# gvtulder/elasticdeform

Hardware: AMD Instinct MI355X
Metric: Mvoxels/s fwd+grad, 256^3 fp32 order=3 (higher is better)
Workload: dtype f32; 1 GPU; cfg2: 3D 256x256x256 float32, 5x5x5 grid sigma 5, order 3, mode mirror, prefilter on, deform_grid + deform_grid_gradient per step, one volume per GPU; parallelism=1 volume per GPU, no collective

## Files before the change

### elasticdeform_amd/csrc/deform_k1z.hip

```cpp
#include <hip/hip_runtime.h>

#include <cstring>
#include <type_traits>

#include "ed_device.h"
#include "ed_gridfilter.h"
#include "ed_params.h"
#include "ed_tile.h"
#include "ed_workspace.h"
#include "ed_zwalk.h"

namespace ed {
namespace tile {

#ifdef EDHIP_K1_STATS
__device__ unsigned long long g_k1z_stats[8];
#define ZSTAT(K, N) atomicAdd(&g_k1z_stats[K], (unsigned long long)(N))
#else
#define ZSTAT(K, N) do { } while (0)
#endif

namespace {


// ... 13 lines not shown
typedef int zv8i __attribute__((ext_vector_type(8)));
typedef const __attribute__((address_space(4))) zv8i* crec_p;
__device__ __forceinline__ ZRecU zrec_unpack(const zv8i& v)
{
    ZRecU r;
    r.b0z = v[0];
    r.b0y = v[1];
    r.b0x = v[2];
    r.flags = v[3];
    r.pitch = (v[3] >> 8) & 255;
    r.ez = v[4] & 1023;
    r.ey = (v[4] >> 10) & 1023;
    r.ex = (int)((unsigned)v[4] >> 20);
    r.goff = v[5];
    r.plane = r.ey * r.pitch;
    return r;
}
__device__ __forceinline__ ZRecU zrec_load(crec_p p)
{
    const zv8i v = *p;
    return zrec_unpack(v);
}

__host__ __device__ __forceinline__ int zctl(int parity, int list, int xcd) { return (parity * 2 + list) * 8 + xcd; }

#define ED_RED6(CTRL)                                      \
    "v_min_i32_dpp %0, %0, %0 " CTRL "\n\t"                \
    "v_min_i32_dpp %1, %1, %1 " CTRL "\n\t"                \
    "v_min_i32_dpp %2, %2, %2 " CTRL "\n\t"                \
    "v_max_i32_dpp %3, %3, %3 " CTRL "\n\t"                \
    "v_max_i32_dpp %4, %4, %4 " CTRL "\n\t"                \
    "v_max_i32_dpp %5, %5, %5 " CTRL "\n\t"
__device__ __forceinline__ void zrow_box(int (&lo)[3], int (&hi)[3])
{
    asm volatile("s_nop 1\n\t"
                 ED_RED6("quad_perm:[1,0,3,2] row_mask:0xf bank_mask:0xf")
                 ED_RED6("quad_perm:[2,3,0,1] row_mask:0xf bank_mask:0xf")
                 ED_RED6("row_half_mirror row_mask:0xf bank_mask:0xf")
                 ED_RED6("row_mirror row_mask:0xf bank_mask:0xf")
                 : "+v"(lo[0]), "+v"(lo[1]), "+v"(lo[2]), "+v"(hi[0]), "+v"(hi[1]), "+v"(hi[2]));
}
#undef ED_RED6
__device__ __forceinline__ int zuni(int v) { return __builtin_amdgcn_readfirstlane(v); }
__device__ __forceinline__ void zlds_barrier() { asm volatile("s_waitcnt lgkmcnt(0)\n\ts_barrier" ::: "memory"); }
__device__ __forceinline__ void zdma_barrier() { asm volatile("s_waitcnt vmcnt(0) lgkmcnt(0)\n\ts_barrier" ::: "memory"); }
__device__ __forceinline__ void zglds16(const float* g, float* lds)
{
    __builtin_amdgcn_global_load_lds((const __attribute__((address_space(1))) void*)g,
                                     (__attribute__((address_space(3))) void*)lds, 16, 0, 0);
}
template <bool OUT16>
__device__ __forceinline__ void zstore_out(float* img, long long off, float val, int io16)
{
    if constexpr (OUT16)
        reinterpret_cast<unsigned short*>(img)[off] = (unsigned short)narrow16(val, io16);
    else
        __builtin_nontemporal_store(val, img + off);
}

__device__ __forceinline__ void zaxis_entry(const GridGeom& g, int a, int oi, double* w, int* idx)
{
    const double cp = control_coordinate(g.ncp[a], (int64_t)oi + g.off[a], g.in_len[a]);
    const int64_t start = window_start(cp, 3);
    const bool edge = start < 0 || start + 3 >= g.ncp[a];
    spline_weights(cp, 3, w);
// ... 3 lines not shown
}

constexpr int kGeoBlock = 256;
constexpr int kGeoWaves = kGeoBlock / 64;
__global__ __launch_bounds__(kGeoBlock) void k1z_geo_kernel(const GridGeom g, const HotGeom hg, const ZGeom zg,
                                                          const GridPrefilter gp)
{
    extern __shared__ __attribute__((aligned(16))) char smem[];
    const int tid = threadIdx.x;
    const int lane = tid & 63;
    const int wave = zuni(tid >> 6);
    const int sample = blockIdx.y;
    const int ncpz = (int)g.ncp[0], ncpy = (int)g.ncp[1], ncpx = (int)g.ncp[2];
    const int nyx = ncpy * ncpx;
    const int ngrid = 3 * ncpz * nyx;
    double* sG = reinterpret_cast<double*>(smem);
    double* sR = sG + ngrid;
    AxTab* sAx = reinterpret_cast<AxTab*>(sR + 64 * ncpz * 3);
    double* sMax = reinterpret_cast<double*>(sAx + 16);
    AxTab* sZ = reinterpret_cast<AxTab*>(sMax + 3 * kGeoWaves);
    int* sCls = reinterpret_cast<int*>(sZ + 4 * hg.tiles[0]);
    int* sBox = sCls + hg.tiles[0];
    int* sCnt = sBox + 64 * hg.tiles[0];
    if ((int)blockIdx.x >= hg.tiles[1] * hg.tiles[2]) {
        const long long nfill = (long long)(gridDim.x - hg.tiles[1] * hg.tiles[2]) * kGeoBlock;
        const long long me = (long long)(blockIdx.x - hg.tiles[1] * hg.tiles[2]) * kGeoBlock + tid;
        const long long n16 = zg.zero_bytes >> 4;
        int4* p16 = reinterpret_cast<int4*>(zg.zero_ptr);
        for (long long i = me; i < n16; i += nfill)
            p16[i] = make_int4(0, 0, 0, 0);
        if (me < (zg.zero_bytes & 15))
            zg.zero_ptr[(n16 << 4) + me] = 0;
        return;
    }
    const int ty = blockIdx.x / hg.tiles[2], tx = blockIdx.x - ty * hg.tiles[2];
    if (ED_DBG(hg.dbg, 1 << 23))
        return;
#ifdef EDHIP_EXPERIMENTS
#define ZTICK(K) do { if (hg.dbgbuf && tid == 0) hg.dbgbuf[(size_t)(blockIdx.x + blockIdx.y * gridDim.x) * 16 + (K)] = __builtin_readcyclecounter(); } while (0)
#else
#define ZTICK(K) do { } while (0)
#endif
    ZTICK(0);

    if (gp.total > 0 && !ED_DBG(hg.dbg, 1 << 28)) {
        grid_prefilter_in_lds<kGeoBlock>(gp, sG, tid);
        if (blockIdx.x == 0 && sample == 0)
            for (int e = tid; e < gp.total; e += kGeoBlock)
                store_cast(gp.out + (int64_t)e * gp.elem_size, gp.dtype, sG[e]);
    } else {
        const char* disp = g.disp + (int64_t)sample * zg.disp_bstride;
        for (int e = tid; e < ngrid; e += kGeoBlock) {
            const int h = e / (ncpz * nyx), r = e - h * (ncpz * nyx);
            const int j0 = r / nyx, j = r - j0 * nyx;
            const int j1 = j / ncpx, j2 = j - j1 * ncpx;
            sG[e] = load_as_double(disp + g.disp_stride[0] * h + g.disp_stride[1] * j0 + g.disp_stride[2] * j1 +
                                       g.disp_stride[3] * j2, g.disp_dtype);
        }
        __syncthreads();
    }
    ZTICK(1);
    if (blockIdx.x == 0 && sample == 0 && tid == 0 && zg.hint) {
        if (zg.hint_host)
            __hip_atomic_store(zg.hint_host, ((unsigned long long)(unsigned)zg.hint[1] << 32) | (unsigned)zg.hint[0],
                               __ATOMIC_RELAXED, __HIP_MEMORY_SCOPE_SYSTEM);
        zg.hint[0] = 0;
        zg.hint[1] = (int)zg.hint_seq;
    }
    for (int h = 0; h < 3 && !ED_DBG(hg.dbg, 1 << 29); ++h) {
        double m = 0.0;
        for (int e = tid; e < ncpz * nyx; e += kGeoBlock)
            m = fmax(m, fabs(sG[h * ncpz * nyx + e]));
        for (int sh = 32; sh >= 1; sh >>= 1)
            m = fmax(m, __shfl_xor(m, sh));
        if (lane == 0)
            sMax[h * kGeoWaves + wave] = m;
    }
    ZTICK(2);
    if (tid < 16 && !ED_DBG(hg.dbg, 1 << 30)) {
        const int a = tid < 8 ? 1 : 2;
        const int oi = min((tid < 8 ? ty : tx) * kT + (tid & 7), hg.out_len[a] - 1);
        AxTab t;
        zaxis_entry(g, a, oi, t.w, t.idx);
        sAx[tid] = t;
    }
    for (int e = tid; e < 4 * hg.tiles[0] && !zg.tables_only && !ED_DBG(hg.dbg, 1 << 26); e += kGeoBlock) {
        const int tz = e >> 2, nz = min(kT, hg.out_len[0] - tz * kT);
        AxTab t;
        zaxis_entry(g, 0, tz * kT + ((e & 3) * (nz - 1)) / 3, t.w, t.idx);
        sZ[e] = t;
    }
    if (blockIdx.x == 0 && sample == 0 && hg.nstep) {
        for (long long ss = tid; ss < hg.nsteps; ss += kGeoBlock) {
            long long vol_off = 0, img_off = 0, r = ss;
            for (int l = 0; l < hg.nstep; ++l) {
                const long long q = r / hg.step_len[l];
                const long long c = r - q * hg.step_len[l];
                vol_off += hg.vol_step[l] * c;
                img_off += hg.img_step[l] * c;
                r = q;
            }
            zg.steps[2 * ss] = vol_off;
            zg.steps[2 * ss + 1] = img_off;
        }
    }
    if (blockIdx.x == 0 && sample == 0 && tid == 0) {
        ZGen* zn = reinterpret_cast<ZGen*>(zg.zgen);
        for (int h = 0; h < 3; ++h) {
            zn->in_len[h] = hg.in_len[h];
            zn->out_len[h] = hg.out_len[h];
            zn->off[h] = hg.off[h];
            zn->period[h] = hg.period[h];
            zn->inv_period[h] = hg.inv_period[h];
            zn->offd[h] = (double)hg.off[h];
        }
        for (int k = 0; k < 12; ++k)
            zn->aff[k] = hg.affine[k];
        zn->mode = hg.mode;
        zn->cval = hg.cval;
        zn->hint = hg.hint;
    }
    if (blockIdx.x == 0 && sample == 0) {
        AxTab* zt = const_cast<AxTab*>(zg.zt);
        for (int oz = tid; oz < hg.out_len[0]; oz += kGeoBlock) {
            AxTab t;
            zaxis_entry(g, 0, oz, t.w, t.idx);
#pragma unroll
            for (int l = 0; l < 4; ++l)
                t.idx[l] *= 32;
            zt[oz] = t;
        }
    }
    __syncthreads();
    ZTICK(3);
    double slack[3];
#pragma unroll
    for (int h = 0; h < 3; ++h) {
        double m = 0.0;
        for (int w = 0; w < kGeoWaves; ++w)
            m = fmax(m, sMax[h * kGeoWaves + w]);
        const double sl = zg.slack_scale * m;
        slack[h] = sl >= 0.02 ? (sl <= 0.75 ? sl : 0.75) : 0.02;
    }
    ZTICK(4);
    if (!ED_DBG(hg.dbg, 1 << 25)) {
        const int col = tid & 63;
        const AxTab ay = sAx[col >> 3];
        const AxTab ax = sAx[8 + (col & 7)];
        int rowoff[4];
#pragma unroll
        for (int ly = 0; ly < 4; ++ly)
            rowoff[ly] = ay.idx[ly] * ncpx;
        for (int r = tid >> 6; r < ncpz * 3; r += kGeoWaves) {
            const int kz = r / 3, h = r - kz * 3;
            const double* gp0 = sG + (h * ncpz + kz) * nyx;
            double acc = 0.0;
#pragma unroll
            for (int ly = 0; ly < 4; ++ly) {
                const double* row = gp0 + rowoff[ly];
                double t = ax.w[0] * row[ax.idx[0]];
#pragma unroll
                for (int lx = 1; lx < 4; ++lx)
                    t = fma(ax.w[lx], row[ax.idx[lx]], t);
                acc = fma(ay.w[ly], t, acc);
            }
            sR[col * (ncpz * 3) + r] = acc;
        }
        __syncthreads();
        double* rg = const_cast<double*>(zg.r) + (int64_t)sample * zg.r_bstride;
        const int rowlen = 8 * 4 * ncpz;
        for (int e = tid; e < 8 * rowlen; e += kGeoBlock) {
            const int py = e / rowlen, j = e - py * rowlen;
            const int px = j / (4 * ncpz), jj = j - px * (4 * ncpz);
            const int kz = jj >> 2, h = jj & 3;
            const int oy = ty * kT + py, ox = tx * kT + px;
            if (oy < hg.out_len[1] && ox < hg.out_len[2])
                rg[((int64_t)oy * hg.out_len[2] + ox) * (4 * ncpz) + jj] = h < 3 ? sR[(py * 8 + px) * (ncpz * 3) + kz * 3 + h] : 0.0;
        }
    }
    if (zg.tables_only)
        return;
    __syncthreads();
    ZTICK(5);
    const int order = zg.order;
    const int H = order / 2, NT = order + 1, kPadX = NT & 1;
    const int ny = min(kT, hg.out_len[1] - ty * kT), nx = min(kT, hg.out_len[2] - tx * kT);
    const int py = (((lane >> 2) & 3) * (ny - 1)) / 3, px = ((lane & 3) * (nx - 1)) / 3;
    const double* rc = sR + (py * 8 + px) * (ncpz * 3);
    for (int tz = wave; tz < hg.tiles[0] && !ED_DBG(hg.dbg, 1 << 24); tz += kGeoWaves) {
        const int nz = min(kT, hg.out_len[0] - tz * kT);
        const int pz = ((lane >> 4) * (nz - 1)) / 3;
        const int o[3] = {tz * kT + pz, ty * kT + py, tx * kT + px};
        const AxTab& ze = sZ[tz * 4 + (lane >> 4)];
        double d[3];
#pragma unroll
        for (int h = 0; h < 3; ++h) {
            d[h] = ze.w[0] * rc[ze.idx[0] * 3 + h];
#pragma unroll
            for (int l = 1; l < 4; ++l)
                d[h] = fma(ze.w[l], rc[ze.idx[l] * 3 + h], d[h]);
        }
        double c[3];
        int lo[3], hi[3];
#pragma unroll
        for (int h = 0; h < 3; ++h) {
// ... 32 lines not shown
                    m = map_coordinate_fast(m, hg.in_len[h], hg.mode, hg.period[h], hg.inv_period[h]);
                cst = cst || !(m > -1.0);
                const double mr = (order & 1) ? m : m + 0.5;
                lo[h] = (int)floor(mr - slack[h]);
                hi[h] = (int)floor(mr + slack[h]);
            }
            if (cst) {
#pragma unroll
                for (int h = 0; h < 3; ++h) {
                    lo[h] = 0x7fffffff;
                    hi[h] = (int)0x80000000;
                }
            }
            zrow_box(lo, hi);
            if ((lane & 15) == 0) {
#pragma unroll
                for (int h = 0; h < 3; ++h) {
                    dst[32 + h] = lo[h];
                    dst[36 + h] = hi[h];
                }
            }
        }
    }
    __syncthreads();
    ZTICK(6);
    for (int tz = tid; tz < hg.tiles[0] && !ED_DBG(hg.dbg, 1 << 27); tz += kGeoBlock) {
        const int tile_id = sample * hg.ntiles + (tz * hg.tiles[1] + ty) * hg.tiles[2] + tx;
        int cls = 0;
        bool hint0 = false, half_fit[2] = {false, false};
#pragma unroll 1
        for (int part = 0; part < 3; ++part) {
            const int* sb = sBox + tz * 64;
            const bool fast = sb[3] != 0;
            const int r0 = part == 2 ? 2 : 0, r1 = part == 1 ? 2 : 3;
            int blo[3], bhi[3];
            bool any = true;
#pragma unroll
            for (int h = 0; h < 3; ++h) {
                int rlo = 0x7fffffff, rhi = (int)0x80000000, lo = 0x7fffffff, hi = (int)0x80000000;
                for (int r = r0; r <= r1; ++r) {
                    rlo = min(rlo, sb[r * 8 + h]);
                    rhi = max(rhi, sb[r * 8 + 4 + h]);
                    lo = min(lo, sb[(fast ? 0 : 32) + r * 8 + h]);
                    hi = max(hi, sb[(fast ? 0 : 32) + r * 8 + 4 + h]);
                }
                if (!fast) {
                    any = any && hi >= lo;
// ... 36 lines not shown
                dst[0] = w0;
                dst[1] = w1;
                if (hg.boxes) {
                    int* bx = hg.boxes + (size_t)tile_id * 8;
#pragma unroll
                    for (int h = 0; h < 3; ++h) {
                        bx[h] = blo[h];
                        bx[3 + h] = bhi[h] - ((h == 2 && any) ? kPadX : 0);
                    }
                }
                if (cls != 3)
                    break;
            } else {
                half_fit[part - 1] = fits || !any;
                int4* dst = reinterpret_cast<int4*>(zg.recs_half + ((size_t)tile_id * 2 + (part - 1)) * 8);
                dst[0] = w0;
                dst[1] = w1;
            }
        }
        const bool split = cls == 3 && half_fit[0] && half_fit[1];
        ZSTAT(cls == 3 ? (split ? 6 : 5) : (cls == 1 ? 3 : 4), 1);
        sCls[tz] = cls | (split ? 4 : 0) | (hint0 ? 8 : 0);
    }
    __syncthreads();
    ZTICK(7);
    {
        const int zstrips = (hg.tiles[0] + zg.strip_tiles - 1) / zg.strip_tiles;
        if (tid < 4)
            sCnt[tid] = 0;
        __syncthreads();
        int slotG = -1, slotF = -1, sidv = 0;
        if (tid < zstrips) {
            int info = 0;
            bool g = false, f = false;
            for (int k = 0; k < zg.strip_tiles && tid * zg.strip_tiles + k < hg.tiles[0]; ++k) {
                const int c = sCls[tid * zg.strip_tiles + k];
                info |= c << (4 * k);
                g = g || (c & 3) == 2 || (c & 7) == 7;
                f = f || (c & 7) == 3;
            }
            const size_t sid = (size_t)sample * zg.nstrips + ((size_t)tid * hg.tiles[1] + ty) * hg.tiles[2] + tx;
            sidv = (int)sid;
            zg.sinfo[sid] = info;
            zg.missed[sid] = f ? 2 : 0;
            if (g)
                slotG = atomicAdd(&sCnt[0], 1);
            if (f)
                slotF = atomicAdd(&sCnt[1], 1);
        }
        __syncthreads();
        const int xcd = (tx + ty + sample) & 7;
        if (tid == 0) {
            sCnt[2] = sCnt[0] ? atomicAdd(&zg.ctl[zctl(zg.parity, 0, xcd)], sCnt[0]) : 0;
            sCnt[3] = sCnt[1] ? atomicAdd(&zg.ctl[zctl(zg.parity, 1, xcd)], sCnt[1]) : 0;
        }
        if (blockIdx.x == 0 && sample == 0 && tid < 16)
            zg.ctl[zctl(1 - zg.parity, tid >> 3, tid & 7)] = 0;
        __syncthreads();
        if (slotG >= 0)
            zg.list_g[(size_t)(sCnt[2] + slotG) * 8 + xcd] = sidv;
        if (slotF >= 0)
            zg.list_f[(size_t)(sCnt[3] + slotF) * 8 + xcd] = sidv;
    }
    ZTICK(8);
#undef ZTICK
}


struct ZVox {
    int addr[2];
    float frac[2][3];
    int flg;
};
struct ZStrip {
    int tz0, ty, tx, ntile, sample, id;
};
__device__ __forceinline__ bool k1z_strip(int total_strips, int nstrips, int tiles_z, int tiles_y, int tiles_x, int strip_tiles, int deal,
                                          ZStrip& sp, int b)
{
    const int x = b & 7, j = b >> 3;
    const int r = j / deal;
    int s = (r * 8 + ((x + r) & 7)) * deal + (j - r * deal);
    if (s >= total_strips)
        return false;
    sp.id = s;
    sp.sample = s / nstrips;
    s -= sp.sample * nstrips;
    sp.tx = s % tiles_x;
    s /= tiles_x;
    sp.ty = s % tiles_y;
    sp.tz0 = (s / tiles_y) * strip_tiles;
    sp.ntile = min(strip_tiles, tiles_z - sp.tz0);
    return true;
}
inline unsigned k1z_grid(int total_strips, int deal)
{
    const int chunks = (total_strips + deal - 1) / deal;
    return (unsigned)(((chunks + 7) / 8) * 8 * deal);
}

template <int ORDER, int PITCH>
__device__ __forceinline__ float k1z_gather(const float* bp, int plane, int pitch_rt, const float* w0, const float* w1, const float* w2)
{
    constexpr int NT = ORDER + 1;
    constexpr int NTX = NT + (NT & 1);
    float a0 = 0.f;
#pragma unroll
    for (int l0 = 0; l0 < NT; ++l0) {
        const float* pp = bp + l0 * plane;
        float a1 = 0.f;
#pragma unroll
        for (int l1 = 0; l1 < NT; ++l1) {
            const float* rp = pp + l1 * (PITCH ? PITCH : pitch_rt);
            float a2 = 0.f;
#pragma unroll
            for (int l2 = 0; l2 < NTX; l2 += 2) {
                const float2 pr = *reinterpret_cast<const float2*>(rp + l2);
                ED_NO_DS_MERGE();
                a2 = fmaf(w2[l2], pr.x, a2);
                a2 = fmaf(w2[l2 + 1], pr.y, a2);
            }
            a1 = fmaf(w1[l1], a2, a1);
        }
// ... 11 lines not shown
    float w0[NT], w1[NT], w2[NTX];
    weights_from_frac<float, ORDER>(f0, w0);
    weights_from_frac<float, ORDER>(f1, w1);
    weights_from_frac<float, ORDER>(f2, w2);
    if (NT & 1)
        w2[NT] = 0.f;
    const float* bp = reinterpret_cast<const float*>(smem + addr);
    return pitch == 16 ? k1z_gather<ORDER, 16>(bp, plane, 16, w0, w1, w2) : k1z_gather<ORDER, 0>(bp, plane, pitch, w0, w1, w2);
}

struct ZFast {
    const float* vol;
    float* img;
    const double* r;
    const AxTab* zt;
    const int* recs;
    const int* recs_half;
    int* missed;
    int* hint;
    const int* sinfo;
    const int* list_g;
    int* list_f;
    int* ctl;
    int parity;
    const long long* steps;
    long long vol_bstride, img_bstride, r_bstride;
    int vol_sy, vol_sz, img_sy, img_sz;
    int box_cap, tiles_y, tiles_x, tiles_z, strip_tiles, nstrips, total_strips, ntiles;
    int rcol_bytes, out_y, out_x;
    int kz0, ky0, kx0;
    int io16, nsteps, deal;
    int dbg;
    double aff[12];
};

template <int ORDER, bool AFFINE, bool OUT16, bool STEPS>
__device__ __forceinline__ void k1z_fast_body(const ZFast& a, const int vblock)
{
    constexpr int NT = ORDER + 1;
    constexpr int kPadX = NT & 1;
    constexpr int NTX = NT + kPadX;
    extern __shared__ __attribute__((aligned(16))) char smem[];
    ZStrip sp;
    if (!k1z_strip(a.total_strips, a.nstrips, a.tiles_z, a.tiles_y, a.tiles_x, a.strip_tiles, a.deal, sp, vblock))
        return;
    const int tid = threadIdx.x;
    const int lane = tid & 63;
// ... 123 lines not shown
        }
        const long long ozoff = (long long)((sp.tz0 + ti) * kT + wave) * img_sz + obase;
        const int nsteps = STEPS ? a.nsteps : 1;
        for (int ss = 0; ss < nsteps; ++ss) {
            if (STEPS && ss > 0)
                stage(rc, vol + steps[2 * ss]);
            zdma_barrier();
#pragma unroll
            for (int i = 0; i < 2; ++i) {
                const float val = ED_DBG(a.dbg, 1 << 17) ? cur.frac[i][0] + cur.frac[i][1] + cur.frac[i][2] + __int_as_float(cur.addr[i])
                                                         : k1z_voxel<ORDER>(smem, cur.addr[i], cur.frac[i], rc.pitch, rc.plane);
                if (!ED_DBG(a.dbg, 1 << 20) || val == 123.456f)
                    zstore_out<OUT16>(img, (STEPS ? steps[2 * ss + 1] : 0) + ozoff + (long long)(4 * i) * img_sz, val, io16);
            }
            zlds_barrier();
        }
        cur = nxt;
        rc = rn;
        ti = tn;
    }
    if (__any(bad < 0) && lane == 0) {
        if (atomicOr(a.missed + sp.id, 1) == 0) {
            const int xcd = vblock & 7;
            a.list_f[(size_t)atomicAdd(a.ctl + zctl(a.parity, 1, xcd), 1) * 8 + xcd] = sp.id;
        }
    }
}

template <int ORDER, bool AFFINE, bool OUT16, bool STEPS>
__device__ __forceinline__ void k1z_gen_body(const ZFast& a, czgen_p zn, const int vblock, const int ngen)
{
    constexpr int NT = ORDER + 1;
    constexpr int kPadX = NT & 1;
    constexpr int NTX = NT + kPadX;
    extern __shared__ __attribute__((aligned(16))) char smem[];
    const int tid = threadIdx.x;
    const int lane = tid & 63;
    const int wave = zuni(tid >> 6);
    const int io16 = OUT16 ? a.io16 : 0;
    const int xcd = vblock & 7, nper = ngen >> 3;
    const int nwork = ((cint_p)(const void*)a.ctl)[zctl(a.parity, 0, xcd)];
    if ((vblock >> 3) >= nwork)
        return;
    const int box_cap = a.box_cap;
    const int odd_shift = (box_cap - 1) * 4;
    float* box0 = reinterpret_cast<float*>(smem);
    float* box1 = box0 + box_cap;
    const int vol_sz = a.vol_sz, vol_sy = a.vol_sy, img_sz = a.img_sz;
    const size_t tile_step = (size_t)a.tiles_y * a.tiles_x;
    cdbl_p zt = (cdbl_p)(const void*)a.zt;
    cll_p steps = (cll_p)(const void*)a.steps;
    const int nsteps = STEPS ? a.nsteps : 1;
    const int yy = lane >> 3, xx = lane & 7;

    for (int work = vblock >> 3; work < nwork; work += nper) {
        ZStrip sp;
        {
            int sid = ((cint_p)(const void*)a.list_g)[(size_t)work * 8 + xcd];
            sp.id = sid;
            sp.sample = sid / a.nstrips;
            sid -= sp.sample * a.nstrips;
            sp.tx = sid % a.tiles_x;
            sid /= a.tiles_x;
            sp.ty = sid % a.tiles_y;
// ... 147 lines not shown
                        stage(rc, vol + steps[2 * ss]);
                    if (staged)
                        zdma_barrier();
#pragma unroll
                    for (int i = 0; i < 2; ++i) {
                        if (!(cur.flg & (4 << i)))
                            continue;
                        float val = zn->cval;
                        if (cur.flg & (1 << i))
                            val = k1z_voxel<ORDER>(smem, cur.addr[i], cur.frac[i], rc.pitch, rc.plane);
                        zstore_out<OUT16>(img, (STEPS ? steps[2 * ss + 1] : 0) + ozoff + (long long)(4 * i) * img_sz, val, io16);
                    }
                    if (staged)
                        zlds_barrier();
                }
                cur = nxt;
                rc = rn;
                it = in;
            }
        }
        if (__any(bad < 0) && lane == 0) {
            if (atomicOr(a.missed + sp.id, 1) == 0) {
                const int xcd = vblock & 7;
                a.list_f[(size_t)atomicAdd(a.ctl + zctl(a.parity, 1, xcd), 1) * 8 + xcd] = sp.id;
            }
        }
    }
}

template <int ORDER, bool AFFINE, bool OUT16, bool STEPS>
__global__ __launch_bounds__(kBlock, 4) void k1z_tile_kernel(const ZFast a, czgen_p zn, const int ngen, const int every)
{
    const int row = (int)(blockIdx.x >> 3), xcd = (int)(blockIdx.x & 7);
    const int gen_rows = ngen >> 3;
    const int gens_before = min((row + 1) / every, gen_rows);
    const bool is_gen = gens_before > 0 && (row + 1) % every == 0 && (row + 1) / every <= gen_rows;
    if (is_gen)
        k1z_gen_body<ORDER, AFFINE, OUT16, STEPS>(a, zn, (gens_before - 1) * 8 + xcd, ngen);
    else
        k1z_fast_body<ORDER, AFFINE, OUT16, STEPS>(a, (row - gens_before) * 8 + xcd);
}

template <int ORDER, bool AFFINE, bool OUT16, bool STEPS>
__global__ __launch_bounds__(kBlock) void k1z_fix_kernel(const ZFast a, czgen_p zn)
{
    constexpr int NT = ORDER + 1;
    constexpr int kPadX = NT & 1;
    const int tid = threadIdx.x;
    const int lane = tid & 63;
    const int wave = zuni(tid >> 6);
    const int io16 = OUT16 ? a.io16 : 0;
    const int xcd = (int)(blockIdx.x & 7), nper = (int)(gridDim.x >> 3);
    const int nwork = ((cint_p)(const void*)a.ctl)[zctl(a.parity, 1, xcd)];
    if ((int)(blockIdx.x >> 3) >= nwork)
        return;
    const int vol_sz = a.vol_sz, vol_sy = a.vol_sy, img_sz = a.img_sz;
    const size_t tile_step = (size_t)a.tiles_y * a.tiles_x;
    cdbl_p zt = (cdbl_p)(const void*)a.zt;
    cll_p steps = (cll_p)(const void*)a.steps;
    const int nsteps = STEPS ? a.nsteps : 1;
    const int yy = lane >> 3, xx = lane & 7;

    for (int work = blockIdx.x >> 3; work < nwork; work += nper) {
        ZStrip sp;
        {
            int sid = ((cint_p)(const void*)a.list_f)[(size_t)work * 8 + xcd];
            sp.id = sid;
            sp.sample = sid / a.nstrips;
            sid -= sp.sample * a.nstrips;
            sp.tx = sid % a.tiles_x;
            sid /= a.tiles_x;
            sp.ty = sid % a.tiles_y;
            sp.tz0 = (sid / a.tiles_y) * a.strip_tiles;
            sp.ntile = min(a.strip_tiles, a.tiles_z - sp.tz0);
        }
        const int ntile = sp.ntile;
// ... 150 lines not shown
{
    const size_t ngrid = 3 * (size_t)g.ncp[0] * (size_t)g.ncp[1] * (size_t)g.ncp[2];
    return 8 * ngrid + 8 * 64 * 3 * (size_t)g.ncp[0] + 16 * sizeof(AxTab) + 3 * kGeoWaves * 8 + (sizeof(AxTab) * 4 + 4 + 256) * (size_t)hg.tiles[0] + 16;
}

size_t k1z_r_bytes(const GridGeom& g) { return 8 * (size_t)g.out_len[1] * (size_t)g.out_len[2] * 4 * (size_t)g.ncp[0]; }

bool k1z_supported(const GridGeom& g)
{
    const size_t ngrid = 3 * (size_t)g.ncp[0] * (size_t)g.ncp[1] * (size_t)g.ncp[2];
    const size_t tiles_z = (size_t)((g.out_len[0] + kT - 1) / kT);
    return ngrid <= 4096 && g.ncp[0] <= 16 &&
           8 * ngrid + 8 * 64 * 3 * (size_t)g.ncp[0] + 16 * sizeof(AxTab) + 3 * kGeoWaves * 8 + (sizeof(AxTab) * 4 + 4 + 256) * tiles_z + 16 <= 60 * 1024;
}

hipError_t launch_k1z_geo(const GridGeom& g, const HotGeom& hg, const ZGeom& zg, const GridPrefilter& gp, int nbatch,
                          hipStream_t stream)
{
    unsigned fill = 0;
    if (zg.zero_ptr && zg.zero_bytes > 0) {
        const long long want = (zg.zero_bytes + 65535) / 65536;
        fill = (unsigned)(want < 1 ? 1 : (want > 2048 ? 2048 : want));
    }
    hipLaunchKernelGGL(k1z_geo_kernel, dim3((unsigned)(hg.tiles[1] * hg.tiles[2]) + fill, (unsigned)nbatch), dim3(kGeoBlock),
                       k1z_geo_lds_bytes(g, hg), stream, g, hg, zg, gp);
    if (ed_env("EDHIP_GEO_TWICE"))
        hipLaunchKernelGGL(k1z_geo_kernel, dim3((unsigned)(hg.tiles[1] * hg.tiles[2]) + fill, (unsigned)nbatch), dim3(kGeoBlock),
                           k1z_geo_lds_bytes(g, hg), stream, g, hg, zg, gp);
    return hipGetLastError();
}

hipError_t launch_k1z(const HotGeom& hg, const ZGeom& zg, int order, size_t lds, hipStream_t stream)
{
    ZFast zf;
    memset(&zf, 0, sizeof(zf));
    zf.vol = hg.vol_r;
    zf.img = hg.img_w;
    zf.r = zg.r;
    zf.zt = zg.zt;
    zf.recs = zg.recs;
    zf.recs_half = zg.recs_half;
    zf.missed = zg.missed;
    zf.hint = hg.hint;
    zf.sinfo = zg.sinfo;
    zf.list_g = zg.list_g;
    zf.list_f = zg.list_f;
    zf.ctl = zg.ctl;
    zf.parity = zg.parity;
    zf.steps = zg.steps;
    zf.vol_bstride = hg.vol_bstride;
    zf.img_bstride = hg.img_bstride;
    zf.r_bstride = zg.r_bstride;
    zf.vol_sy = hg.vol_sy;
    zf.vol_sz = hg.vol_sz;
    zf.img_sy = hg.img_sy;
    zf.img_sz = hg.img_sz;
    zf.box_cap = hg.box_cap;
    zf.tiles_z = hg.tiles[0];
    zf.tiles_y = hg.tiles[1];
    zf.tiles_x = hg.tiles[2];
    zf.strip_tiles = zg.strip_tiles;
    zf.nstrips = zg.nstrips;
    zf.total_strips = zg.total_strips;
    zf.ntiles = hg.ntiles;
    zf.rcol_bytes = 32 * zg.ncpz;
    zf.out_y = hg.out_len[1];
    zf.out_x = hg.out_len[2];
    const int H = order / 2;
    zf.kz0 = (hg.has_affine ? 0 : hg.off[0]) - H;
    zf.ky0 = (hg.has_affine ? 0 : hg.off[1]) - H;
    zf.kx0 = (hg.has_affine ? 0 : hg.off[2]) - H;
// ... 39 lines not shown
```

### elasticdeform_amd/csrc/deform_tile.hip

```cpp
#include <atomic>
#include <type_traits>
#include <cstdint>
#include <cstdlib>
#include <cstring>

#include "ed_device.h"
#include "ed_exact_coord.h"
#include "ed_params.h"
#include "ed_gridfilter.h"
#include "ed_workspace.h"
#include "ed_tile.h"

#ifdef EDHIP_EXPERIMENTS
__device__ unsigned g_wide_clamped;
extern "C" unsigned edhip_debug_wide_clamped(void)
{
    unsigned v = 0xffffffffu, z = 0;
    if (hipMemcpyFromSymbol(&v, HIP_SYMBOL(g_wide_clamped), sizeof(v)) != hipSuccess)
        return 0xffffffffu;
    (void)hipMemcpyToSymbol(HIP_SYMBOL(g_wide_clamped), &z, sizeof(z));
    return v;
}
#endif

// ... 1449 lines not shown
                    double r2 = 0.0;
                    for (int k = 0; k < 3; ++k) {
                        const double r = g.in_len[k] > 1 ? (double)(g.ncp[k] - 1) / (double)(g.in_len[k] - 1) : 0.0;
                        r2 += r * r;
                    }
                    zg.slack_scale = 0.15 * 1.125 * 4.0 * r2;
                    zgeo = geo_buffer(stream);
                    char* gb = zgeo ? (char*)geo_reserve(stream, zgeo, k1z_geo_bytes(g, ntiles, nb), &e) : nullptr;
                    if (!gb)
                        return e != hipSuccess ? e : hipErrorOutOfMemory;
                    zg.ctl = (int*)gb;
                    zg.zgen = gb + 4096;
                    char* zx = gb + 4096 + 512;
                    zg.zt = (const AxTab*)zx;
                    zg.recs = (int*)(zx + k1z_zt_bytes(g));
                    zg.missed = zg.recs + (size_t)ntiles * nb * 8;
                    zg.sinfo = zg.missed + (size_t)ntiles * nb;
                    zg.list_g = zg.sinfo + (size_t)ntiles * nb;
                    zg.list_f = zg.list_g + (size_t)ntiles * nb * 8;
                    zg.recs_half = zg.list_f + (size_t)ntiles * nb * 8;
                    zg.steps = (long long*)(zx + k1z_zt_bytes(g) + (((size_t)ntiles * nb * 168 + 63) & ~(size_t)63));
                    zg.r = (const double*)((char*)zg.steps + kK1zMaxSteps * 16);
                    zg.r_bstride = (long long)(((k1z_r_bytes(g) + 63) & ~(size_t)63) / 8);
                    zg.parity = (int)(zgeo->parity & 1);
                    zg.disp_bstride = tg.disp_bstride;
                    zg.ncpz = (int)g.ncp[0];
                    zg.order = ORDER;
                    zg.strip_tiles = 4;
                    auto zstrips = [&](int st) { return (int64_t)nb * tg.tiles[1] * tg.tiles[2] * ((tg.tiles[0] + st - 1) / st); };
                    if (zstrips(4) < 4096)
                        zg.strip_tiles = 2;
                    if (zstrips(2) < 1024)
                        zg.strip_tiles = 1;
#ifdef EDHIP_EXPERIMENTS
                    if (const char* st = ed_env("EDHIP_ZSTRIP"))
                        zg.strip_tiles = atoi(st) >= 1 ? atoi(st) : zg.strip_tiles;
#endif
                    zg.nstrips = tg.tiles[1] * tg.tiles[2] * ((tg.tiles[0] + zg.strip_tiles - 1) / zg.strip_tiles);
                    zg.total_strips = zg.nstrips * nb;
                    zg.hint = hg.hint;
                    zg.hint_host = tg.hint_host;
                    zg.hint_seq = tg.hint_seq;
#ifdef EDHIP_EXPERIMENTS
                    if (const char* pp = ed_env("EDHIP_DEBUG_PTR"))
                        hg.dbgbuf = (unsigned long long*)strtoull(pp, nullptr, 16);
#endif
                } else if (k1_new) {
// ... 99 lines not shown
                            } else {
                                *key = KeepKey();
                            }
                            rec_route = true;
                        } else if (GRAD && box_mode == 2 && ORDER >= 3 && memcmp(key, &cur, sizeof(cur)) == 0) {
                            hg.boxes = kb;
                            hg.use_boxes = 1;
                            if (self_serve_boxes && ORDER <= 3)
                                hg.self_serve = 1;
                        }
                    }
                }
                if (k1z && e == hipSuccess) {
                    GridPrefilter gp;
                    memset(&gp, 0, sizeof(gp));
                    const bool own = batch && batch->gridpf && nb == 1 && batch->gridpf->total <= 4096;
                    if (own) {
                        gp = *batch->gridpf;
                        gp.zero_ptr = nullptr;
                        gp.zero_bytes = 0;
                    }
                    if (!tables_done && e == hipSuccess) {
                        e = launch_k1z_geo(g, hg, zg, gp, nb, stream);
                        if (e == hipSuccess)
                            ++zgeo->parity;
                        if (own && e == hipSuccess)
                            batch->gridpf_done = true;
                        tables_done = true;
                    }
                }
                bool k2z = false;
#ifdef EDHIP_EXPERIMENTS
                if constexpr (GRAD && ORDER <= 3) {
                    k2z = hlds && !rec_route && !wide && !v.out16 && hg.self_serve && k1z_supported(g) &&
                          ve.nsteps <= (int64_t)kK1zMaxSteps && (ed_env("EDHIP_K2Z") || ed_env("EDHIP_K2Y") || ed_env("EDHIP_K2S")) &&
                          !ed_env("EDHIP_WAVE") && e == hipSuccess;
                }
#endif
                size_t k2lds = 0;
                if (k2z) {
                    zgeo = geo_buffer(stream);
                    char* gb = zgeo ? (char*)geo_reserve(stream, zgeo, k1z_geo_bytes(g, ntiles, nb), &e) : nullptr;
                    if (!gb)
                        return e != hipSuccess ? e : hipErrorOutOfMemory;
                    zg.ctl = (int*)gb;
                    zg.zgen = gb + 4096;
                    char* zx = gb + 4096 + 512;
                    zg.zt = (const AxTab*)zx;
// ... 435 lines not shown
```

### elasticdeform_amd/csrc/ed_tile.h

```cpp
#pragma once

#include "ed_device.h"
#include "ed_params.h"
#include "ed_workspace.h"

namespace ed {
namespace tile {

constexpr int kT = 8;
constexpr int kStrip = 8;
constexpr int kBlock = 256;

struct AxTab {
    double w[4];
    int idx[4];
};

struct __attribute__((packed, aligned(4))) F4u {
    float x, y, z, w;
};
static_assert(sizeof(AxTab) == 48, "AxTab layout");

#define ED_NO_DS_MERGE() asm volatile("" ::: "memory")

// ... 341 lines not shown
constexpr unsigned kRecDead = 0x80000000u;

hipError_t launch_hot_level1(const HotGeom& hg, int order, bool gradient, unsigned nblk, size_t lds,
                             hipStream_t stream);
size_t hot_lds_bytes(bool gradient, int ncpx, int* box_cap, int* off_box, int level = 0);
hipError_t launch_hot_records(const HotGeom& hg, int order, unsigned nblk, size_t lds, hipStream_t stream);
size_t hot_grad2_lds_bytes(int* box_cap, bool large = false);
hipError_t launch_hot_grad2(const HotGeom& hg, int order, unsigned nblk, size_t lds, hipStream_t stream);

size_t k1_lds_bytes(int ncpx, int* box_cap, int* off_box, bool large = false);
hipError_t launch_k1_level1(const HotGeom& hg, int order, unsigned nblk, size_t lds, hipStream_t stream);

struct ZGeom {
    const double* r;
    const AxTab* zt;
    int* recs;
    int* recs_half;
    int* missed;
    long long* steps;
    int* sinfo;
    int* list_g;
    int* list_f;
    int* ctl;
    int parity;
    void* zgen;
    int tables_only;
    char* zero_ptr;
    long long zero_bytes;
    long long r_bstride;
    long long disp_bstride;
    int ncpz;
    int order;
    int strip_tiles;
    int nstrips;
    int total_strips;
    double slack_scale;
    int* hint;
    unsigned long long* hint_host;
    unsigned hint_seq;
};
size_t k1z_lds_bytes(int* box_cap, bool large = false);
bool k1z_supported(const GridGeom& g);
size_t k1z_r_bytes(const GridGeom& g);
hipError_t launch_k1z_geo(const GridGeom& g, const HotGeom& hg, const ZGeom& zg, const GridPrefilter& gp, int nbatch,
                          hipStream_t stream);
hipError_t launch_k1z(const HotGeom& hg, const ZGeom& zg, int order, size_t lds, hipStream_t stream);
size_t k2z_lds_bytes(int* box_cap);
// ... 11 lines not shown
```

### elasticdeform_amd/csrc/ed_workspace.h

```cpp
#pragma once

#include <hip/hip_runtime.h>

#include <cstddef>

namespace ed {

void* workspace_reserve(hipStream_t stream, size_t bytes, hipError_t* err);

struct KeepKey {
    unsigned long long w[48];
};
void* keep_reserve(hipStream_t stream, size_t bytes, KeepKey** key, hipError_t* err);

struct SpillHint {
    volatile unsigned long long* host = nullptr;
    unsigned long long* dev = nullptr;
    unsigned seq = 0;
    struct Call { unsigned seq; unsigned long long key; unsigned tiles; } ring[8] = {};
    struct Entry { unsigned long long key; float frac; } table[8] = {};
    int nring = 0, ntable = 0;

    void absorb();
    float fraction(unsigned long long key) const;
    bool known(unsigned long long key) const;
    unsigned begin_call(unsigned long long key, unsigned tiles);
};
SpillHint* spill_hint(hipStream_t stream);

struct GridStamp {
    const void* raw = nullptr;
    const void* ws = nullptr;
    unsigned long long generation = 0;
    int dtype = 0, ndim = 0;
    long long shape[9] = {}, stride[9] = {};
};
GridStamp* grid_stamp(hipStream_t stream);
unsigned long long workspace_generation(hipStream_t stream);

struct GeoBuffer {
    unsigned parity = 0;
    void* ptr = nullptr;
    size_t cap = 0;
};
GeoBuffer* geo_buffer(hipStream_t stream);
void* geo_reserve(hipStream_t stream, GeoBuffer* geo, size_t bytes, hipError_t* err);

void workspace_release_all();

void workspace_trim(hipStream_t stream);

class StreamGuard {
public:
    explicit StreamGuard(hipStream_t stream);
    ~StreamGuard();
    StreamGuard(const StreamGuard&) = delete;
    StreamGuard& operator=(const StreamGuard&) = delete;

private:
    void* mutex_;
    hipStream_t stream_;
};

}
// ... 1 lines not shown
```

Baseline: 26030 Mvoxels/s.

## Move geo-kernel singleton work to a dedicated block and track list parity on device

The once-per-call work (prefiltered grid store, hint update, step table, ZGen fill, z axis table) moves out of patch block 0 into an extra dedicated block, so block 0 no longer carries serial extra work. The host-side parity counter is replaced by a device-side epoch stored in ctl: the geo kernel reads the next epoch and a later kernel advances it, so list counts are chosen by device state. It also fuses the three per-axis max reductions into one pass using DPP/readlane, replaces one integer division with float reciprocals, and swaps several __syncthreads for lighter LDS-only barriers. Risks include ordering of epoch reads and writes across kernels, and float-reciprocal index rounding errors.

```diff
diff --git a/elasticdeform_amd/csrc/deform_k1z.hip b/elasticdeform_amd/csrc/deform_k1z.hip
--- a/elasticdeform_amd/csrc/deform_k1z.hip
+++ b/elasticdeform_amd/csrc/deform_k1z.hip
@@ -59,7 +59,8 @@
     return zrec_unpack(v);
 }
 
-__host__ __device__ __forceinline__ int zctl(int parity, int list, int xcd) { return (parity * 2 + list) * 8 + xcd; }
+__host__ __device__ __forceinline__ int zctl(int set, int list, int xcd) { return (set * 2 + list) * 8 + xcd; }
+enum : int { kZEpochNext = 32, kZEpochCall = 33 };
 
 #define ED_RED6(CTRL)                                      \
     "v_min_i32_dpp %0, %0, %0 " CTRL "\n\t"                \
@@ -78,6 +79,30 @@
                  : "+v"(lo[0]), "+v"(lo[1]), "+v"(lo[2]), "+v"(hi[0]), "+v"(hi[1]), "+v"(hi[2]));
 }
 #undef ED_RED6
+template <int CTRL>
+__device__ __forceinline__ double zdpp_max_step(double m)
+{
+    const long long b = __double_as_longlong(m);
+    const int lo = __builtin_amdgcn_update_dpp(0, (int)b, CTRL, 0xf, 0xf, false);
+    const int hi = __builtin_amdgcn_update_dpp(0, (int)(b >> 32), CTRL, 0xf, 0xf, false);
+    return fmax(m, __longlong_as_double(((long long)hi << 32) | (unsigned)lo));
+}
+__device__ __forceinline__ double zwave_max(double m)
+{
+    m = zdpp_max_step<0xB1>(m);
+    m = zdpp_max_step<0x4E>(m);
+    m = zdpp_max_step<0x141>(m);
+    m = zdpp_max_step<0x140>(m);
+    const long long b = __double_as_longlong(m);
+    double r = 0.0;
+#pragma unroll
+    for (int row = 0; row < 4; ++row) {
+        const int lo = __builtin_amdgcn_readlane((int)b, row * 16);
+        const int hi = __builtin_amdgcn_readlane((int)(b >> 32), row * 16);
+        r = fmax(r, __longlong_as_double(((long long)hi << 32) | (unsigned)lo));
+    }
+    return r;
+}
 __device__ __forceinline__ int zuni(int v) { return __builtin_amdgcn_readfirstlane(v); }
 __device__ __forceinline__ void zlds_barrier() { asm volatile("s_waitcnt lgkmcnt(0)\n\ts_barrier" ::: "memory"); }
 __device__ __forceinline__ void zdma_barrier() { asm volatile("s_waitcnt vmcnt(0) lgkmcnt(0)\n\ts_barrier" ::: "memory"); }
@@ -127,15 +152,78 @@
     int* sCls = reinterpret_cast<int*>(sZ + 4 * hg.tiles[0]);
     int* sBox = sCls + hg.tiles[0];
     int* sCnt = sBox + 64 * hg.tiles[0];
-    if ((int)blockIdx.x >= hg.tiles[1] * hg.tiles[2]) {
-        const long long nfill = (long long)(gridDim.x - hg.tiles[1] * hg.tiles[2]) * kGeoBlock;
-        const long long me = (long long)(blockIdx.x - hg.tiles[1] * hg.tiles[2]) * kGeoBlock + tid;
+    const int npatch = hg.tiles[1] * hg.tiles[2];
+    if ((int)blockIdx.x > npatch) {
+        const long long nfill = (long long)(gridDim.x - npatch - 1) * kGeoBlock;
+        const long long me = (long long)(blockIdx.x - npatch - 1) * kGeoBlock + tid;
         const long long n16 = zg.zero_bytes >> 4;
         int4* p16 = reinterpret_cast<int4*>(zg.zero_ptr);
         for (long long i = me; i < n16; i += nfill)
             p16[i] = make_int4(0, 0, 0, 0);
         if (me < (zg.zero_bytes & 15))
             zg.zero_ptr[(n16 << 4) + me] = 0;
+        return;
+    }
+    if ((int)blockIdx.x == npatch) {
+        if (sample != 0)
+            return;
+        if (gp.total > 0 && !ED_DBG(hg.dbg, 1 << 28)) {
+            grid_prefilter_in_lds<kGeoBlock>(gp, sG, tid);
+            for (int e = tid; e < gp.total; e += kGeoBlock)
+                store_cast(gp.out + (int64_t)e * gp.elem_size, gp.dtype, sG[e]);
+        }
+        if (tid == 0 && zg.hint) {
+            if (zg.hint_host)
+                __hip_atomic_store(zg.hint_host, ((unsigned long long)(unsigned)zg.hint[1] << 32) | (unsigned)zg.hint[0],
+                                   __ATOMIC_RELAXED, __HIP_MEMORY_SCOPE_SYSTEM);
+            zg.hint[0] = 0;
+            zg.hint[1] = (int)zg.hint_seq;
+        }
+        if (tid < 16) {
+            const int epoch = zg.ctl[kZEpochNext];
+            zg.ctl[zctl(1 - (epoch & 1), tid >> 3, tid & 7)] = 0;
+            if (tid == 0)
+                zg.ctl[kZEpochCall] = epoch;
+        }
+        if (hg.nstep) {
+            for (long long ss = tid; ss < hg.nsteps; ss += kGeoBlock) {
+                long long vol_off = 0, img_off = 0, r = ss;
+                for (int l = 0; l < hg.nstep; ++l) {
+                    const long long q = r / hg.step_len[l];
+                    const long long c = r - q * hg.step_len[l];
+                    vol_off += hg.vol_step[l] * c;
+                    img_off += hg.img_step[l] * c;
+                    r = q;
+                }
+                zg.steps[2 * ss] = vol_off;
+                zg.steps[2 * ss + 1] = img_off;
+            }
+        }
+        if (tid == 0) {
+            ZGen* zn = reinterpret_cast<ZGen*>(zg.zgen);
+            for (int h = 0; h < 3; ++h) {
+                zn->in_len[h] = hg.in_len[h];
+                zn->out_len[h] = hg.out_len[h];
+                zn->off[h] = hg.off[h];
+                zn->period[h] = hg.period[h];
+                zn->inv_period[h] = hg.inv_period[h];
+                zn->offd[h] = (double)hg.off[h];
+            }
+            for (int k = 0; k < 12; ++k)
+                zn->aff[k] = hg.affine[k];
+            zn->mode = hg.mode;
+            zn->cval = hg.cval;
+            zn->hint = hg.hint;
+        }
+        AxTab* zt = const_cast<AxTab*>(zg.zt);
+        for (int oz = tid; oz < hg.out_len[0]; oz += kGeoBlock) {
+            AxTab t;
+            zaxis_entry(g, 0, oz, t.w, t.idx);
+#pragma unroll
+            for (int l = 0; l < 4; ++l)
+                t.idx[l] *= 32;
+            zt[oz] = t;
+        }
         return;
     }
     const int ty = blockIdx.x / hg.tiles[2], tx = blockIdx.x - ty * hg.tiles[2];
@@ -147,12 +235,10 @@
 #define ZTICK(K) do { } while (0)
 #endif
     ZTICK(0);
+    const int cset = zg.tables_only ? 0 : (((cint_p)(const void*)zg.ctl)[kZEpochNext] & 1);
 
     if (gp.total > 0 && !ED_DBG(hg.dbg, 1 << 28)) {
         grid_prefilter_in_lds<kGeoBlock>(gp, sG, tid);
-        if (blockIdx.x == 0 && sample == 0)
-            for (int e = tid; e < gp.total; e += kGeoBlock)
-                store_cast(gp.out + (int64_t)e * gp.elem_size, gp.dtype, sG[e]);
     } else {
         const char* disp = g.disp + (int64_t)sample * zg.disp_bstride;
         for (int e = tid; e < ngrid; e += kGeoBlock) {
@@ -165,76 +251,34 @@
         __syncthreads();
     }
     ZTICK(1);
-    if (blockIdx.x == 0 && sample == 0 && tid == 0 && zg.hint) {
-        if (zg.hint_host)
-            __hip_atomic_store(zg.hint_host, ((unsigned long long)(unsigned)zg.hint[1] << 32) | (unsigned)zg.hint[0],
-                               __ATOMIC_RELAXED, __HIP_MEMORY_SCOPE_SYSTEM);
-        zg.hint[0] = 0;
-        zg.hint[1] = (int)zg.hint_seq;
-    }
-    for (int h = 0; h < 3 && !ED_DBG(hg.dbg, 1 << 29); ++h) {
-        double m = 0.0;
-        for (int e = tid; e < ncpz * nyx; e += kGeoBlock)
-            m = fmax(m, fabs(sG[h * ncpz * nyx + e]));
-        for (int sh = 32; sh >= 1; sh >>= 1)
-            m = fmax(m, __shfl_xor(m, sh));
-        if (lane == 0)
-            sMax[h * kGeoWaves + wave] = m;
+    if (!ED_DBG(hg.dbg, 1 << 29)) {
+        double m[3] = {0.0, 0.0, 0.0};
+        for (int e = tid; e < ncpz * nyx; e += kGeoBlock) {
+#pragma unroll
+            for (int h = 0; h < 3; ++h)
+                m[h] = fmax(m[h], fabs(sG[h * ncpz * nyx + e]));
+        }
+#pragma unroll
+        for (int h = 0; h < 3; ++h) {
+            m[h] = zwave_max(m[h]);
+            if (lane == 0)
+                sMax[h * kGeoWaves + wave] = m[h];
+        }
     }
     ZTICK(2);
-    if (tid < 16 && !ED_DBG(hg.dbg, 1 << 30)) {
-        const int a = tid < 8 ? 1 : 2;
-        const int oi = min((tid < 8 ? ty : tx) * kT + (tid & 7), hg.out_len[a] - 1);
+    if (tid >= kGeoBlock - 16 && !ED_DBG(hg.dbg, 1 << 30)) {
+        const int k = tid - (kGeoBlock - 16);
+        const int a = k < 8 ? 1 : 2;
+        const int oi = min((k < 8 ? ty : tx) * kT + (k & 7), hg.out_len[a] - 1);
         AxTab t;
         zaxis_entry(g, a, oi, t.w, t.idx);
-        sAx[tid] = t;
+        sAx[k] = t;
     }
     for (int e = tid; e < 4 * hg.tiles[0] && !zg.tables_only && !ED_DBG(hg.dbg, 1 << 26); e += kGeoBlock) {
         const int tz = e >> 2, nz = min(kT, hg.out_len[0] - tz * kT);
         AxTab t;
         zaxis_entry(g, 0, tz * kT + ((e & 3) * (nz - 1)) / 3, t.w, t.idx);
         sZ[e] = t;
-    }
-    if (blockIdx.x == 0 && sample == 0 && hg.nstep) {
-        for (long long ss = tid; ss < hg.nsteps; ss += kGeoBlock) {
-            long long vol_off = 0, img_off = 0, r = ss;
-            for (int l = 0; l < hg.nstep; ++l) {
-                const long long q = r / hg.step_len[l];
-                const long long c = r - q * hg.step_len[l];
-                vol_off += hg.vol_step[l] * c;
-                img_off += hg.img_step[l] * c;
-                r = q;
-            }
-            zg.steps[2 * ss] = vol_off;
-            zg.steps[2 * ss + 1] = img_off;
-        }
-    }
-    if (blockIdx.x == 0 && sample == 0 && tid == 0) {
-        ZGen* zn = reinterpret_cast<ZGen*>(zg.zgen);
-        for (int h = 0; h < 3; ++h) {
-            zn->in_len[h] = hg.in_len[h];
-            zn->out_len[h] = hg.out_len[h];
-            zn->off[h] = hg.off[h];
-            zn->period[h] = hg.period[h];
-            zn->inv_period[h] = hg.inv_period[h];
-            zn->offd[h] = (double)hg.off[h];
-        }
-        for (int k = 0; k < 12; ++k)
-            zn->aff[k] = hg.affine[k];
-        zn->mode = hg.mode;
-        zn->cval = hg.cval;
-        zn->hint = hg.hint;
-    }
-    if (blockIdx.x == 0 && sample == 0) {
-        AxTab* zt = const_cast<AxTab*>(zg.zt);
-        for (int oz = tid; oz < hg.out_len[0]; oz += kGeoBlock) {
-            AxTab t;
-            zaxis_entry(g, 0, oz, t.w, t.idx);
-#pragma unroll
-            for (int l = 0; l < 4; ++l)
-                t.idx[l] *= 32;
-            zt[oz] = t;
-        }
     }
     __syncthreads();
     ZTICK(3);
@@ -274,9 +318,10 @@
         __syncthreads();
         double* rg = const_cast<double*>(zg.r) + (int64_t)sample * zg.r_bstride;
         const int rowlen = 8 * 4 * ncpz;
+        const float inv_rowlen = __frcp_rn((float)rowlen), inv_col = __frcp_rn((float)(4 * ncpz));
         for (int e = tid; e < 8 * rowlen; e += kGeoBlock) {
-            const int py = e / rowlen, j = e - py * rowlen;
-            const int px = j / (4 * ncpz), jj = j - px * (4 * ncpz);
+            const int py = (int)(((float)e + 0.5f) * inv_rowlen), j = e - py * rowlen;
+            const int px = (int)(((float)j + 0.5f) * inv_col), jj = j - px * (4 * ncpz);
             const int kz = jj >> 2, h = jj & 3;
             const int oy = ty * kT + py, ox = tx * kT + px;
             if (oy < hg.out_len[1] && ox < hg.out_len[2])
@@ -285,7 +330,6 @@
     }
     if (zg.tables_only)
         return;
-    __syncthreads();
     ZTICK(5);
     const int order = zg.order;
     const int H = order / 2, NT = order + 1, kPadX = NT & 1;
@@ -364,7 +408,7 @@
             }
         }
     }
-    __syncthreads();
+    zlds_barrier();
     ZTICK(6);
     for (int tz = tid; tz < hg.tiles[0] && !ED_DBG(hg.dbg, 1 << 27); tz += kGeoBlock) {
         const int tile_id = sample * hg.ntiles + (tz * hg.tiles[1] + ty) * hg.tiles[2] + tx;
@@ -447,13 +491,13 @@
         ZSTAT(cls == 3 ? (split ? 6 : 5) : (cls == 1 ? 3 : 4), 1);
         sCls[tz] = cls | (split ? 4 : 0) | (hint0 ? 8 : 0);
     }
-    __syncthreads();
+    zlds_barrier();
     ZTICK(7);
     {
         const int zstrips = (hg.tiles[0] + zg.strip_tiles - 1) / zg.strip_tiles;
         if (tid < 4)
             sCnt[tid] = 0;
-        __syncthreads();
+        zlds_barrier();
         int slotG = -1, slotF = -1, sidv = 0;
         if (tid < zstrips) {
             int info = 0;
@@ -473,15 +517,11 @@
             if (f)
                 slotF = atomicAdd(&sCnt[1], 1);
         }
-        __syncthreads();
+        zlds_barrier();
         const int xcd = (tx + ty + sample) & 7;
-        if (tid == 0) {
-            sCnt[2] = sCnt[0] ? atomicAdd(&zg.ctl[zctl(zg.parity, 0, xcd)], sCnt[0]) : 0;
-            sCnt[3] = sCnt[1] ? atomicAdd(&zg.ctl[zctl(zg.parity, 1, xcd)], sCnt[1]) : 0;
-        }
-        if (blockIdx.x == 0 && sample == 0 && tid < 16)
-            zg.ctl[zctl(1 - zg.parity, tid >> 3, tid & 7)] = 0;
-        __syncthreads();
+        if (lane == 0 && wave < 2)
+            sCnt[2 + wave] = sCnt[wave] ? atomicAdd(&zg.ctl[zctl(cset, wave, xcd)], sCnt[wave]) : 0;
+        zlds_barrier();
         if (slotG >= 0)
             zg.list_g[(size_t)(sCnt[2] + slotG) * 8 + xcd] = sidv;
         if (slotF >= 0)
@@ -524,6 +564,13 @@
     return (unsigned)(((chunks + 7) / 8) * 8 * deal);
 }
 
+__device__ __forceinline__ int k1z_count(const int* ctl, int list, int xcd)
+{
+    cint_p c = (cint_p)(const void*)ctl;
+    const int n0 = c[zctl(0, list, xcd)], n1 = c[zctl(1, list, xcd)], epoch = c[kZEpochCall];
+    return (epoch & 1) ? n1 : n0;
+}
+
 template <int ORDER, int PITCH>
 __device__ __forceinline__ float k1z_gather(const float* bp, int plane, int pitch_rt, const float* w0, const float* w1, const float* w2)
 {
@@ -581,7 +628,6 @@
     const int* list_g;
     int* list_f;
     int* ctl;
-    int parity;
     const long long* steps;
     long long vol_bstride, img_bstride, r_bstride;
     int vol_sy, vol_sz, img_sy, img_sz;
@@ -751,7 +797,8 @@
     if (__any(bad < 0) && lane == 0) {
         if (atomicOr(a.missed + sp.id, 1) == 0) {
             const int xcd = vblock & 7;
-            a.list_f[(size_t)atomicAdd(a.ctl + zctl(a.parity, 1, xcd), 1) * 8 + xcd] = sp.id;
+            const int cset = ((cint_p)(const void*)a.ctl)[kZEpochCall] & 1;
+            a.list_f[(size_t)atomicAdd(a.ctl + zctl(cset, 1, xcd), 1) * 8 + xcd] = sp.id;
         }
     }
 }
@@ -768,7 +815,7 @@
     const int wave = zuni(tid >> 6);
     const int io16 = OUT16 ? a.io16 : 0;
     const int xcd = vblock & 7, nper = ngen >> 3;
-    const int nwork = ((cint_p)(const void*)a.ctl)[zctl(a.parity, 0, xcd)];
+    const int nwork = k1z_count(a.ctl, 0, xcd);
     if ((vblock >> 3) >= nwork)
         return;
     const int box_cap = a.box_cap;
@@ -962,7 +1009,8 @@
         if (__any(bad < 0) && lane == 0) {
             if (atomicOr(a.missed + sp.id, 1) == 0) {
                 const int xcd = vblock & 7;
-                a.list_f[(size_t)atomicAdd(a.ctl + zctl(a.parity, 1, xcd), 1) * 8 + xcd] = sp.id;
+                const int cset = ((cint_p)(const void*)a.ctl)[kZEpochCall] & 1;
+                a.list_f[(size_t)atomicAdd(a.ctl + zctl(cset, 1, xcd), 1) * 8 + xcd] = sp.id;
             }
         }
     }
@@ -973,6 +1021,8 @@
 {
     const int row = (int)(blockIdx.x >> 3), xcd = (int)(blockIdx.x & 7);
     const int gen_rows = ngen >> 3;
+    if (blockIdx.x == 0 && threadIdx.x == 0)
+        a.ctl[kZEpochNext] = (((cint_p)(const void*)a.ctl)[kZEpochCall] + 1) & 1;
     const int gens_before = min((row + 1) / every, gen_rows);
     const bool is_gen = gens_before > 0 && (row + 1) % every == 0 && (row + 1) / every <= gen_rows;
     if (is_gen)
@@ -991,7 +1041,7 @@
     const int wave = zuni(tid >> 6);
     const int io16 = OUT16 ? a.io16 : 0;
     const int xcd = (int)(blockIdx.x & 7), nper = (int)(gridDim.x >> 3);
-    const int nwork = ((cint_p)(const void*)a.ctl)[zctl(a.parity, 1, xcd)];
+    const int nwork = k1z_count(a.ctl, 1, xcd);
     if ((int)(blockIdx.x >> 3) >= nwork)
         return;
     const int vol_sz = a.vol_sz, vol_sy = a.vol_sy, img_sz = a.img_sz;
@@ -1188,10 +1238,10 @@
         const long long want = (zg.zero_bytes + 65535) / 65536;
         fill = (unsigned)(want < 1 ? 1 : (want > 2048 ? 2048 : want));
     }
-    hipLaunchKernelGGL(k1z_geo_kernel, dim3((unsigned)(hg.tiles[1] * hg.tiles[2]) + fill, (unsigned)nbatch), dim3(kGeoBlock),
+    hipLaunchKernelGGL(k1z_geo_kernel, dim3((unsigned)(hg.tiles[1] * hg.tiles[2]) + 1 + fill, (unsigned)nbatch), dim3(kGeoBlock),
                        k1z_geo_lds_bytes(g, hg), stream, g, hg, zg, gp);
     if (ed_env("EDHIP_GEO_TWICE"))
-        hipLaunchKernelGGL(k1z_geo_kernel, dim3((unsigned)(hg.tiles[1] * hg.tiles[2]) + fill, (unsigned)nbatch), dim3(kGeoBlock),
+        hipLaunchKernelGGL(k1z_geo_kernel, dim3((unsigned)(hg.tiles[1] * hg.tiles[2]) + 1 + fill, (unsigned)nbatch), dim3(kGeoBlock),
                            k1z_geo_lds_bytes(g, hg), stream, g, hg, zg, gp);
     return hipGetLastError();
 }
@@ -1212,7 +1262,6 @@
     zf.list_g = zg.list_g;
     zf.list_f = zg.list_f;
     zf.ctl = zg.ctl;
-    zf.parity = zg.parity;
     zf.steps = zg.steps;
     zf.vol_bstride = hg.vol_bstride;
     zf.img_bstride = hg.img_bstride;
diff --git a/elasticdeform_amd/csrc/deform_tile.hip b/elasticdeform_amd/csrc/deform_tile.hip
--- a/elasticdeform_amd/csrc/deform_tile.hip
+++ b/elasticdeform_amd/csrc/deform_tile.hip
@@ -1495,7 +1495,6 @@
                     zg.steps = (long long*)(zx + k1z_zt_bytes(g) + (((size_t)ntiles * nb * 168 + 63) & ~(size_t)63));
                     zg.r = (const double*)((char*)zg.steps + kK1zMaxSteps * 16);
                     zg.r_bstride = (long long)(((k1z_r_bytes(g) + 63) & ~(size_t)63) / 8);
-                    zg.parity = (int)(zgeo->parity & 1);
                     zg.disp_bstride = tg.disp_bstride;
                     zg.ncpz = (int)g.ncp[0];
                     zg.order = ORDER;
@@ -1641,8 +1640,6 @@
                     }
                     if (!tables_done && e == hipSuccess) {
                         e = launch_k1z_geo(g, hg, zg, gp, nb, stream);
-                        if (e == hipSuccess)
-                            ++zgeo->parity;
                         if (own && e == hipSuccess)
                             batch->gridpf_done = true;
                         tables_done = true;
diff --git a/elasticdeform_amd/csrc/ed_tile.h b/elasticdeform_amd/csrc/ed_tile.h
--- a/elasticdeform_amd/csrc/ed_tile.h
+++ b/elasticdeform_amd/csrc/ed_tile.h
@@ -387,7 +387,6 @@
     int* list_g;
     int* list_f;
     int* ctl;
-    int parity;
     void* zgen;
     int tables_only;
     char* zero_ptr;
diff --git a/elasticdeform_amd/csrc/ed_workspace.h b/elasticdeform_amd/csrc/ed_workspace.h
--- a/elasticdeform_amd/csrc/ed_workspace.h
+++ b/elasticdeform_amd/csrc/ed_workspace.h
@@ -39,7 +39,6 @@
 unsigned long long workspace_generation(hipStream_t stream);
 
 struct GeoBuffer {
-    unsigned parity = 0;
     void* ptr = nullptr;
     size_t cap = 0;
 };
```

After: 26040 Mvoxels/s, median of 5. About the same (+0.0%).
